# songxf1024/GIMS

Hardware: NVIDIA B200
Metric: image_pairs_per_sec_2048kp (higher is better)
Workload: dtype f32

## Files before the change

gims_b200/csrc/attention_f16.cu:

```cuda
#include <math_constants.h>

#include "common.cuh"
#include "tc_common.cuh"

namespace gims {

namespace {

using namespace tc;

constexpr int TQ = 128;
constexpr int NQT = 2;
constexpr int TKV = 64;
constexpr int HD = 64;
constexpr int kStages = 4;
constexpr int kPlaneBytes = TKV * HD * 2;
constexpr int kThreads16 = 384;

template <int PLANES> struct Cfg16 {
  static constexpr int kStageBytes = PLANES * kPlaneBytes;
  static constexpr int kSmem = 2 * kStages * kStageBytes + 1024 + 512;
};

constexpr int cS = 0, cPh = 64, cPl = 96, cO = 128, cQh = 192, cQl = 224, cTile = 256;

__device__ long long* g_attn16_trace = nullptr;

struct Attn16Args {
  const float* qp;
  float* out;
  Segs segs;
  int cross;
  int rows_total;
  int vbase[kMaxSegs];
  unsigned* status;
};

__device__ __forceinline__ float ex2_approx(float x) {
  float y;
  asm("ex2.approx.ftz.f32 %0, %1;" : "=f"(y) : "f"(x));
  return y;
}

__device__ __forceinline__ uint64_t uniform64(uint64_t x) {
  const uint32_t lo = __shfl_sync(0xffffffffu, (uint32_t)x, 0), hi = __shfl_sync(0xffffffffu, (uint32_t)(x >> 32), 0);
  return ((uint64_t)hi << 32) | lo;
}

template <int PLANES, int FMT>
__global__ void __launch_bounds__(kThreads16, 1)
k_attention_f16(const __grid_constant__ CUtensorMap mapK, const __grid_constant__ CUtensorMap mapVt, Attn16Args a) {
  extern __shared__ uint8_t smem_raw[];
  using Cfg = Cfg16<PLANES>;
  const int img = blockIdx.z, head = blockIdx.y;
  const int src = a.cross ? (img ^ 1) : img;
  const int nq = __shfl_sync(0xffffffffu, seg_count(a.segs, img), 0);
  const int nk = __shfl_sync(0xffffffffu, seg_count(a.segs, src), 0);
  const int q0 = blockIdx.x * (NQT * TQ);
  if (q0 >= nq || nk <= 0) return;
  const int nqt = (q0 + TQ < nq) ? 2 : 1;
  const int qrow0 = a.segs.base[img] + q0;
  const int krow0 = a.segs.base[src];
  const int ntiles = (nk + TKV - 1) / TKV;

  uint8_t* smem = reinterpret_cast<uint8_t*>((reinterpret_cast<uintptr_t>(smem_raw) + 1023) & ~uintptr_t(1023));
  uint8_t* k_smem = smem;
  uint8_t* v_smem = k_smem + kStages * Cfg::kStageBytes;
  uint64_t* bars = reinterpret_cast<uint64_t*>(v_smem + kStages * Cfg::kStageBytes);
  uint64_t* k_full = bars;
  uint64_t* k_empty = bars + kStages;
  uint64_t* v_full = bars + 2 * kStages;
  uint64_t* v_empty = bars + 3 * kStages;
  uint64_t* s_full = bars + 4 * kStages;
  uint64_t* s_free = s_full + 2;
  uint64_t* p_full = s_free + 2;
  uint64_t* o_full = p_full + 2;
  uint64_t* o_free = o_full + 2;
  uint64_t* q_ready = o_free + 2;
  uint64_t* skew = q_ready + 2;
  uint32_t* tmem_slot = reinterpret_cast<uint32_t*>(skew + 1);


  const int warp = threadIdx.x >> 5, lane = threadIdx.x & 31;
  constexpr int kWarpQk = 8, kWarpPv = 9;
  if (warp == kWarpQk && lane == 0) {
    tma_prefetch_desc(&mapK);
    tma_prefetch_desc(&mapVt);
    for (int s = 0; s < kStages; ++s) {
      mbar_init(&k_full[s], 1); mbar_init(&k_empty[s], nqt);
      mbar_init(&v_full[s], 1); mbar_init(&v_empty[s], nqt);
    }
    for (int t = 0; t < 2; ++t) {
      mbar_init(&s_full[t], 1); mbar_init(&s_free[t], 4);
      mbar_init(&p_full[t], 4); mbar_init(&o_full[t], 1); mbar_init(&o_free[t], 4);
      mbar_init(&q_ready[t], 4);
    }
    mbar_init(skew, 4);
    fence_barrier_init();
  }
  const int qt = warp >> 2;
  float4 qreg[HD / 4];
  if (warp < 8) {
    const int qr = q0 + TQ * qt + 32 * (warp & 3) + lane;
    const float4* p4 = reinterpret_cast<const float4*>(a.qp + (size_t)(qrow0 + TQ * qt + 32 * (warp & 3) + lane) * kD + head * HD);
#pragma unroll
    for (int i = 0; i < HD / 4; ++i) qreg[i] = (qr < nq) ? p4[i] : make_float4(0.f, 0.f, 0.f, 0.f);
  }
  if (warp == kWarpQk) tmem_alloc<512>(tmem_slot);
  tcgen05_fence_before();
  __syncthreads();
  tcgen05_fence_after();
  const uint32_t tmem = __shfl_sync(0xffffffffu, *tmem_slot, 0);

  const int wt = __shfl_sync(0xffffffffu, (warp - kWarpQk) >> 1, 0);
  if (warp >= 8) {
    if ((threadIdx.x == kWarpQk * 32 || threadIdx.x == (kWarpQk + 2) * 32) && wt < nqt) {
      const int t = wt;
      constexpr uint32_t idesc = umma_idesc_f16(TQ, TKV, FMT);
      const uint64_t dk0 = umma_desc_sw128(smem_u32(k_smem));
      const uint32_t sacc = tmem + cTile * t + cS, q_hi = tmem + cTile * t + cQh, q_lo = tmem + cTile * t + cQl;
      auto load_k = [&](int j, int s) {
        mbar_arrive_expect_tx(&k_full[s], Cfg::kStageBytes);
        for (int pl = 0; pl < PLANES; ++pl)
          tma_load_2d(k_smem + s * Cfg::kStageBytes + pl * kPlaneBytes, &mapK, &k_full[s], head * HD, pl * a.rows_total + krow0 + j * TKV);
      };
      if (t == 0)
        for (int j = 0; j < kStages && j < ntiles; ++j) load_k(j, j);
      mbar_wait(&q_ready[t], 0);
      long long* trace = (blockIdx.x | blockIdx.y | blockIdx.z) == 0 && t == 0 ? g_attn16_trace : nullptr;
      int s = 0; uint32_t ph = 0;
      for (int j = 0; j < ntiles; ++j) {
        mbar_wait(&k_full[s], ph);
        if (j > 0) mbar_wait(&s_free[t], (uint32_t)(j - 1) & 1u);
        tcgen05_fence_after();
        if (trace && j < 40) trace[j * 16 + 0] = clock64();
        const uint64_t kh = dk0 + (uint64_t)(s * (Cfg::kStageBytes >> 4)), kl = kh + (kPlaneBytes >> 4);
        if (PLANES == 2) {
#pragma unroll
          for (int ks = 0; ks < 4; ++ks) {
            umma_f16_ts(sacc, q_lo + ks * 8, kh + ks * 2, idesc, ks ? 1u : 0u);
            umma_f16_ts(sacc, q_hi + ks * 8, kl + ks * 2, idesc, 1u);
          }
        }
#pragma unroll
        for (int ks = 0; ks < 4; ++ks) umma_f16_ts(sacc, q_hi + ks * 8, kh + ks * 2, idesc, (PLANES == 2 || ks) ? 1u : 0u);
        umma_commit(&s_full[t]);
        umma_commit(&k_empty[s]);
        if (trace && j < 40) trace[j * 16 + 1] = clock64();
        if (t == 0 && j >= 1 && j - 1 + kStages < ntiles) {
          const int sp = s == 0 ? kStages - 1 : s - 1;
          mbar_wait(&k_empty[sp], (uint32_t)((j - 1) / kStages) & 1u);
          load_k(j - 1 + kStages, sp);
        }
        if (++s == kStages) { s = 0; ph ^= 1; }
      }
    } else if ((threadIdx.x == kWarpPv * 32 || threadIdx.x == (kWarpPv + 2) * 32) && wt < nqt) {
      const int t = wt;
      constexpr uint32_t idesc = umma_idesc_f16(TQ, HD, FMT);
      const uint64_t dv0 = umma_desc_sw128(smem_u32(v_smem));
      const uint32_t oacc = tmem + cTile * t + cO, p_hi = tmem + cTile * t + cPh, p_lo = tmem + cTile * t + cPl;
      auto load_v = [&](int j, int s) {
        mbar_arrive_expect_tx(&v_full[s], Cfg::kStageBytes);
        for (int pl = 0; pl < PLANES; ++pl)
          tma_load_2d(v_smem + s * Cfg::kStageBytes + pl * kPlaneBytes, &mapVt, &v_full[s], a.vbase[src] + j * TKV, pl * kD + head * HD);
      };
      if (t == 0)
        for (int j = 0; j < kStages && j < ntiles; ++j) load_v(j, j);
      long long* trace = (blockIdx.x | blockIdx.y | blockIdx.z) == 0 && t == 0 ? g_attn16_trace : nullptr;
      int s = 0; uint32_t ph = 0;
      for (int j = 0; j < ntiles; ++j) {
        mbar_wait(&v_full[s], ph);
        mbar_wait(&p_full[t], (uint32_t)j & 1u);
        if (j > 0) mbar_wait(&o_free[t], (uint32_t)(j - 1) & 1u);
        tcgen05_fence_after();
        if (trace && j < 40) trace[j * 16 + 2] = clock64();
        const uint64_t vh = dv0 + (uint64_t)(s * (Cfg::kStageBytes >> 4)), vl = vh + (kPlaneBytes >> 4);
        if (PLANES == 2) {
#pragma unroll
          for (int ks = 0; ks < 4; ++ks) {
            umma_f16_ts(oacc, p_lo + ks * 8, vh + ks * 2, idesc, ks ? 1u : 0u);
            umma_f16_ts(oacc, p_hi + ks * 8, vl + ks * 2, idesc, 1u);
          }
        }
#pragma unroll
        for (int ks = 0; ks < 4; ++ks) umma_f16_ts(oacc, p_hi + ks * 8, vh + ks * 2, idesc, (PLANES == 2 || ks) ? 1u : 0u);
        umma_commit(&o_full[t]);
        umma_commit(&v_empty[s]);
        if (trace && j < 40) trace[j * 16 + 3] = clock64();
        if (t == 0 && j >= 1 && j - 1 + kStages < ntiles) {
          const int sp = s == 0 ? kStages - 1 : s - 1;
          mbar_wait(&v_empty[sp], (uint32_t)((j - 1) / kStages) & 1u);
          load_v(j - 1 + kStages, sp);
        }
        if (++s == kStages) { s = 0; ph ^= 1; }
      }
    }
  } else {
    if (qt < nqt) {
      const uint32_t lane_base = tmem + ((uint32_t)(32 * (warp & 3)) << 16) + (uint32_t)(cTile * qt);
      const int row = q0 + TQ * qt + 32 * (warp & 3) + lane;
      bool ovf = false;
      {
        uint32_t vh[32], vl[32];
#pragma unroll
        for (int i = 0; i < HD / 4; ++i) {
          const float4 x = qreg[i];
          if (FMT == 0) ovf = ovf || fmaxf(fmaxf(fabsf(x.x), fabsf(x.y)), fmaxf(fabsf(x.z), fabsf(x.w))) >= 32768.f;
          if (PLANES == 2) {
            split16x2<FMT>(x.x, x.y, vh[2 * i], vl[2 * i]);
            split16x2<FMT>(x.z, x.w, vh[2 * i + 1], vl[2 * i + 1]);
          } else {
            vh[2 * i] = pack16<FMT>(x.x, x.y);
            vh[2 * i + 1] = pack16<FMT>(x.z, x.w);
          }
        }
        tmem_st_32x32(lane_base + cQh, vh);
        if (PLANES == 2) tmem_st_32x32(lane_base + cQl, vl);
        tmem_st_wait();
        tcgen05_fence_before();
        __syncwarp();
        if (lane == 0) mbar_arrive(&q_ready[qt]);
      }
      if (__any_sync(0xffffffffu, ovf) && lane == 0 && a.status) atomicOr(a.status, GIMS_STATUS_FP16_RANGE);
      float o[HD];
#pragma unroll
      for (int d = 0; d < HD; ++d) o[d] = 0.f;
      float m_run = -CUDART_INF_F, l_run = 0.f, alpha_prev = 0.f;
      long long* trace = ((blockIdx.x | blockIdx.y | blockIdx.z) == 0 && (threadIdx.x & 127) == 0) ? g_attn16_trace : nullptr;
      for (int j = 0; j <= ntiles; ++j) {
        float s[TKV];
        float alpha = 0.f;
        uint32_t ph_[32], pl_[32];
        if (j < ntiles) {
          if (j == 0 && qt == 1) mbar_wait(skew, 0);
          mbar_wait(&s_full[qt], (uint32_t)j & 1u);
          tcgen05_fence_after();
          if (trace && j < 40) trace[j * 16 + (qt ? 7 : 4)] = clock64();
          {
            uint32_t v0[32], v1[32];
            tmem_ld_32x32(lane_base + cS, v0);
            tmem_ld_32x32(lane_base + cS + 32, v1);
            tmem_ld_wait();
#pragma unroll
            for (int i = 0; i < 32; ++i) { s[i] = __uint_as_float(v0[i]); s[32 + i] = __uint_as_float(v1[i]); }
          }
          tcgen05_fence_before();
          __syncwarp();
          if (lane == 0) mbar_arrive(&s_free[qt]);
          if (trace && j < 40 && qt == 0) trace[j * 16 + 8] = clock64();
          const int valid = nk - j * TKV;
          if (valid < TKV) {
#pragma unroll
            for (int i = 0; i < TKV; ++i)
              if (i >= valid) s[i] = -CUDART_INF_F;
          }
          float mx8[8];
#pragma unroll
          for (int i = 0; i < 8; ++i) mx8[i] = s[i];
#pragma unroll
          for (int i = 8; i < TKV; ++i) mx8[i & 7] = fmaxf(mx8[i & 7], s[i]);
          const float mx = fmaxf(fmaxf(fmaxf(mx8[0], mx8[1]), fmaxf(mx8[2], mx8[3])), fmaxf(fmaxf(mx8[4], mx8[5]), fmaxf(mx8[6], mx8[7])));
          const float m_new = fmaxf(m_run, mx);
          if (trace && j < 40 && qt == 0) trace[j * 16 + 9] = clock64() + (long long)(__float_as_int(m_new) & 0);
          alpha = ex2_approx(m_run - m_new);
          float rs[4] = {0.f, 0.f, 0.f, 0.f};
#pragma unroll
          for (int i = 0; i < TKV; i += 4) {
#pragma unroll
            for (int q = 0; q < 4; ++q) {
              s[i + q] = ex2_approx(s[i + q] - m_new);
              rs[q] += s[i + q];
            }
          }
          l_run = l_run * alpha + ((rs[0] + rs[1]) + (rs[2] + rs[3]));
          m_run = m_new;
          if (trace && j < 40 && qt == 0) trace[j * 16 + 10] = clock64() + (long long)(__float_as_int(l_run) & 0);
          if (j == 0 && qt == 0) { __syncwarp(); if (lane == 0) mbar_arrive(skew); }
#pragma unroll
          for (int i = 0; i < 32; ++i) {
            if (PLANES == 2) split16x2<FMT>(s[2 * i], s[2 * i + 1], ph_[i], pl_[i]);
            else ph_[i] = pack16<FMT>(s[2 * i], s[2 * i + 1]);
          }
        }
        if (j > 0) {
          mbar_wait(&o_full[qt], (uint32_t)(j - 1) & 1u);
          tcgen05_fence_after();
          if (trace && j < 40 && qt == 0) trace[j * 16 + 11] = clock64();
        }
        if (j < ntiles) {
          tmem_st_32x32(lane_base + cPh, ph_);
          if (PLANES == 2) tmem_st_32x32(lane_base + cPl, pl_);
          tmem_st_wait();
          tcgen05_fence_before();
          __syncwarp();
          if (lane == 0) mbar_arrive(&p_full[qt]);
          if (trace && j < 40 && qt == 0) trace[j * 16 + 5] = clock64();
        }
        if (j > 0) {
          {
            uint32_t v0[32], v1[32];
            tmem_ld_32x32(lane_base + cO, v0);
            tmem_ld_32x32(lane_base + cO + 32, v1);
            tmem_ld_wait();
#pragma unroll
            for (int i = 0; i < 32; ++i) {
              o[i] = fmaf(o[i], alpha_prev, __uint_as_float(v0[i]));
              o[32 + i] = fmaf(o[32 + i], alpha_prev, __uint_as_float(v1[i]));
            }
          }
          tcgen05_fence_before();
          __syncwarp();
          if (lane == 0) mbar_arrive(&o_free[qt]);
          if (trace && j < 40 && qt == 0) trace[j * 16 + 6] = clock64();
        }
        alpha_prev = alpha;
      }
      if (row < nq) {
        const float inv = 1.f / l_run;
        float4* dst = reinterpret_cast<float4*>(a.out + (size_t)(a.segs.base[img] + row) * kD + head * HD);
#pragma unroll
        for (int d = 0; d < HD; d += 4) dst[d / 4] = make_float4(o[d] * inv, o[d + 1] * inv, o[d + 2] * inv, o[d + 3] * inv);
      }
      tcgen05_fence_before();
    }
  }
  __syncthreads();
  if (warp == kWarpQk) {
    tcgen05_fence_after();
    tmem_dealloc<512>(tmem);
  }
}

template <int PLANES, int FMT>
int launch16(const CUtensorMap& mK, const CUtensorMap& mV, const Attn16Args& a, dim3 grid, cudaStream_t st) {
  using Cfg = Cfg16<PLANES>;
  GIMS_CUDA_OK(cudaFuncSetAttribute(k_attention_f16<PLANES, FMT>, cudaFuncAttributeMaxDynamicSharedMemorySize, Cfg::kSmem));
  k_attention_f16<PLANES, FMT><<<grid, kThreads16, Cfg::kSmem, st>>>(mK, mV, a);
  GIMS_LAUNCH_OK();
  return GIMS_OK;
}

}

int set_attention16_trace(long long* dev_buf) {
  GIMS_CUDA_OK(cudaMemcpyToSymbol(g_attn16_trace, &dev_buf, sizeof(dev_buf)));
  return GIMS_OK;
}

int launch_attention_f16(const QkvPlanes& pl, float* out, const Segs& segs, int cross, cudaStream_t st) {
  const int rows = segs_rows(segs);
  if (pl.fmt < 0 || (pl.planes != 1 && pl.planes != 2) || pl.ldv % 8) {
    set_error("launch_attention_f16: bad plane description (fmt %d, planes %d, ldv %d)", pl.fmt, pl.planes, pl.ldv);
    return GIMS_ERR_ARG;
  }
  CUtensorMap mK, mV;
  GIMS_TRY(tc::make_tmap_16_k64(&mK, pl.kp, pl.fmt, (uint64_t)pl.planes * rows, kD, kD, TKV));
  GIMS_TRY(tc::make_tmap_16_k64(&mV, pl.vt, pl.fmt, (uint64_t)pl.planes * kD, pl.ldv, pl.ldv, HD));
  Attn16Args a;
  a.qp = pl.qp;
  a.out = out;
  a.segs = segs;
  a.cross = cross;
  a.rows_total = rows;
  for (int i = 0; i < kMaxSegs; ++i) a.vbase[i] = pl.vbase[i];
  a.status = pl.status;
  dim3 grid(cdiv(segs_nmax(segs), NQT * TQ), kHeads, segs.nseg);
  ProfScope prof(GIMS_PROF_ATTENTION, st);
  if (pl.planes == 2 && pl.fmt == 0) return launch16<2, 0>(mK, mV, a, grid, st);
  if (pl.planes == 1 && pl.fmt == 1) return launch16<1, 1>(mK, mV, a, grid, st);
  set_error("launch_attention_f16: unsupported combination planes=%d fmt=%d", pl.planes, pl.fmt);
  return GIMS_ERR_ARG;
}

}
```

gims_b200/csrc/tc_common.cuh:

```cuda
#pragma once
#include <cuda.h>
#include <cuda_runtime.h>
#include <stdint.h>

namespace gims {
namespace tc {

__device__ __forceinline__ uint32_t smem_u32(const void* p) { return (uint32_t)__cvta_generic_to_shared(p); }

__device__ __forceinline__ void mbar_init(uint64_t* bar, uint32_t count) {
  asm volatile("mbarrier.init.shared::cta.b64 [%0], %1;" ::"r"(smem_u32(bar)), "r"(count) : "memory");
}
__device__ __forceinline__ void fence_barrier_init() { asm volatile("fence.mbarrier_init.release.cluster;" ::: "memory"); }
__device__ __forceinline__ void mbar_arrive(uint64_t* bar) {
  asm volatile("mbarrier.arrive.shared::cta.b64 _, [%0];" ::"r"(smem_u32(bar)) : "memory");
}
__device__ __forceinline__ void mbar_arrive_expect_tx(uint64_t* bar, uint32_t bytes) {
  asm volatile("mbarrier.arrive.expect_tx.shared::cta.b64 _, [%0], %1;" ::"r"(smem_u32(bar)), "r"(bytes) : "memory");
}
static __device__ unsigned g_tc_timeout_flag;
static __device__ unsigned g_tc_timeout_info[4];
__device__ __forceinline__ bool mbar_try_wait(uint32_t addr, uint32_t parity) {
  uint32_t ok;
  asm volatile(
      "{\n\t.reg .pred p;\n\t"
      "mbarrier.try_wait.parity.shared::cta.b64 p, [%1], %2;\n\t"
      "selp.u32 %0, 1, 0, p;\n\t}"
      : "=r"(ok)
      : "r"(addr), "r"(parity)
      : "memory");
  return ok != 0;
}
__device__ __forceinline__ void mbar_wait(uint64_t* bar, uint32_t parity) {
  const uint32_t addr = smem_u32(bar);
  unsigned spins = 0;
  while (!mbar_try_wait(addr, parity)) {
    if (++spins > 400000u || ((spins & 255u) == 0 && *(volatile unsigned*)&g_tc_timeout_flag)) {
      if (atomicExch(&g_tc_timeout_flag, 1u) == 0u) {
        g_tc_timeout_info[0] = blockIdx.x; g_tc_timeout_info[1] = blockIdx.y | (blockIdx.z << 16);
        g_tc_timeout_info[2] = threadIdx.x; g_tc_timeout_info[3] = addr | (parity << 31);
      }
      return;
    }
  }
}

__device__ __forceinline__ void fence_proxy_async_smem() { asm volatile("fence.proxy.async.shared::cta;" ::: "memory"); }
__device__ __forceinline__ void tcgen05_fence_before() { asm volatile("tcgen05.fence::before_thread_sync;" ::: "memory"); }
__device__ __forceinline__ void tcgen05_fence_after() { asm volatile("tcgen05.fence::after_thread_sync;" ::: "memory"); }

__device__ __forceinline__ void tma_prefetch_desc(const CUtensorMap* m) {
  asm volatile("prefetch.tensormap [%0];" ::"l"(reinterpret_cast<uint64_t>(m)) : "memory");
}
__device__ __forceinline__ void tma_load_2d(void* smem_dst, const CUtensorMap* m, uint64_t* bar, int c0, int c1) {
  asm volatile(
      "cp.async.bulk.tensor.2d.shared::cluster.global.mbarrier::complete_tx::bytes [%0], [%1, {%3, %4}], [%2];" ::"r"(
          smem_u32(smem_dst)),
      "l"(reinterpret_cast<uint64_t>(m)), "r"(smem_u32(bar)), "r"(c0), "r"(c1)
      : "memory");
}

template <int COLS>
__device__ __forceinline__ void tmem_alloc(uint32_t* smem_result) {
  static_assert(COLS == 32 || COLS == 64 || COLS == 128 || COLS == 256 || COLS == 512, "TMEM columns: power of 2 >= 32");
  asm volatile("tcgen05.alloc.cta_group::1.sync.aligned.shared::cta.b32 [%0], %1;" ::"r"(smem_u32(smem_result)), "n"(COLS)
               : "memory");
  asm volatile("tcgen05.relinquish_alloc_permit.cta_group::1.sync.aligned;" ::: "memory");
}
template <int COLS>
__device__ __forceinline__ void tmem_dealloc(uint32_t taddr) {
  asm volatile("tcgen05.dealloc.cta_group::1.sync.aligned.b32 %0, %1;" ::"r"(taddr), "n"(COLS) : "memory");
}

__device__ __forceinline__ void tmem_ld_32x32(uint32_t taddr, uint32_t (&r)[32]) {
  asm volatile(
      "tcgen05.ld.sync.aligned.32x32b.x32.b32 "
      "{%0, %1, %2, %3, %4, %5, %6, %7, %8, %9, %10, %11, %12, %13, %14, %15, "
      "%16, %17, %18, %19, %20, %21, %22, %23, %24, %25, %26, %27, %28, %29, %30, %31}, [%32];"
      : "=r"(r[0]), "=r"(r[1]), "=r"(r[2]), "=r"(r[3]), "=r"(r[4]), "=r"(r[5]), "=r"(r[6]), "=r"(r[7]), "=r"(r[8]),
        "=r"(r[9]), "=r"(r[10]), "=r"(r[11]), "=r"(r[12]), "=r"(r[13]), "=r"(r[14]), "=r"(r[15]), "=r"(r[16]),
        "=r"(r[17]), "=r"(r[18]), "=r"(r[19]), "=r"(r[20]), "=r"(r[21]), "=r"(r[22]), "=r"(r[23]), "=r"(r[24]),
        "=r"(r[25]), "=r"(r[26]), "=r"(r[27]), "=r"(r[28]), "=r"(r[29]), "=r"(r[30]), "=r"(r[31])
      : "r"(taddr)
      : "memory");
}
__device__ __forceinline__ void tmem_ld_wait() { asm volatile("tcgen05.wait::ld.sync.aligned;" ::: "memory"); }

__device__ __forceinline__ uint64_t umma_desc_sw128(uint32_t smem_addr) {
  uint64_t d = 0;
  d |= (uint64_t)((smem_addr >> 4) & 0x3FFF);
  d |= (uint64_t)1 << 16;
  d |= (uint64_t)64 << 32;
  d |= (uint64_t)1 << 46;
  d |= (uint64_t)2 << 61;
  return d;
}
__host__ __device__ constexpr uint32_t umma_idesc_tf32(int m, int n) {
  return (1u << 4) | (2u << 7) | (2u << 10) | ((uint32_t)(n >> 3) << 17) | ((uint32_t)(m >> 4) << 24);
}
__device__ __forceinline__ void umma_tf32_ss(uint32_t tmem_d, uint64_t desc_a, uint64_t desc_b, uint32_t idesc,
                                             uint32_t accumulate) {
  asm volatile(
      "{\n\t.reg .pred p;\n\t"
      "setp.ne.b32 p, %4, 0;\n\t"
      "tcgen05.mma.cta_group::1.kind::tf32 [%0], %1, %2, %3, p;\n\t}" ::"r"(tmem_d),
      "l"(desc_a), "l"(desc_b), "r"(idesc), "r"(accumulate)
      : "memory");
}
__device__ __forceinline__ void tmem_st_32x32(uint32_t taddr, const uint32_t (&r)[32]) {
  asm volatile(
      "tcgen05.st.sync.aligned.32x32b.x32.b32 [%0], "
      "{%1, %2, %3, %4, %5, %6, %7, %8, %9, %10, %11, %12, %13, %14, %15, %16, "
      "%17, %18, %19, %20, %21, %22, %23, %24, %25, %26, %27, %28, %29, %30, %31, %32};" ::"r"(taddr),
      "r"(r[0]), "r"(r[1]), "r"(r[2]), "r"(r[3]), "r"(r[4]), "r"(r[5]), "r"(r[6]), "r"(r[7]), "r"(r[8]), "r"(r[9]),
      "r"(r[10]), "r"(r[11]), "r"(r[12]), "r"(r[13]), "r"(r[14]), "r"(r[15]), "r"(r[16]), "r"(r[17]), "r"(r[18]),
      "r"(r[19]), "r"(r[20]), "r"(r[21]), "r"(r[22]), "r"(r[23]), "r"(r[24]), "r"(r[25]), "r"(r[26]), "r"(r[27]),
      "r"(r[28]), "r"(r[29]), "r"(r[30]), "r"(r[31])
      : "memory");
}
__device__ __forceinline__ void tmem_st_32x16(uint32_t taddr, const uint32_t (&r)[16]) {
  asm volatile(
      "tcgen05.st.sync.aligned.32x32b.x16.b32 [%0], "
      "{%1, %2, %3, %4, %5, %6, %7, %8, %9, %10, %11, %12, %13, %14, %15, %16};" ::"r"(taddr),
      "r"(r[0]), "r"(r[1]), "r"(r[2]), "r"(r[3]), "r"(r[4]), "r"(r[5]), "r"(r[6]), "r"(r[7]), "r"(r[8]), "r"(r[9]),
      "r"(r[10]), "r"(r[11]), "r"(r[12]), "r"(r[13]), "r"(r[14]), "r"(r[15])
      : "memory");
}
__device__ __forceinline__ void tmem_st_wait() { asm volatile("tcgen05.wait::st.sync.aligned;" ::: "memory"); }

__device__ __forceinline__ void umma_tf32_ts(uint32_t tmem_d, uint32_t tmem_a, uint64_t desc_b, uint32_t idesc,
                                             uint32_t accumulate) {
  asm volatile(
      "{\n\t.reg .pred p;\n\t"
      "setp.ne.b32 p, %4, 0;\n\t"
      "tcgen05.mma.cta_group::1.kind::tf32 [%0], [%1], %2, %3, p;\n\t}" ::"r"(tmem_d),
      "r"(tmem_a), "l"(desc_b), "r"(idesc), "r"(accumulate)
      : "memory");
}
__host__ __device__ constexpr uint32_t umma_idesc_f16(int m, int n, int fmt) {
  return (1u << 4) | ((uint32_t)fmt << 7) | ((uint32_t)fmt << 10) | ((uint32_t)(n >> 3) << 17) | ((uint32_t)(m >> 4) << 24);
}
__device__ __forceinline__ void umma_f16_ts(uint32_t tmem_d, uint32_t tmem_a, uint64_t desc_b, uint32_t idesc,
                                            uint32_t accumulate) {
  asm volatile(
      "{\n\t.reg .pred p;\n\t"
      "setp.ne.b32 p, %4, 0;\n\t"
      "tcgen05.mma.cta_group::1.kind::f16 [%0], [%1], %2, %3, p;\n\t}" ::"r"(tmem_d),
      "r"(tmem_a), "l"(desc_b), "r"(idesc), "r"(accumulate)
      : "memory");
}
template <int FMT>
__device__ __forceinline__ uint32_t pack16(float lo, float hi) {
  uint32_t d;
  if (FMT == 0) asm("cvt.rn.f16x2.f32 %0, %1, %2;" : "=r"(d) : "f"(hi), "f"(lo));
  else          asm("cvt.rn.bf16x2.f32 %0, %1, %2;" : "=r"(d) : "f"(hi), "f"(lo));
  return d;
}
template <int FMT>
__device__ __forceinline__ void unpack16(uint32_t d, float& lo, float& hi) {
  if (FMT == 0) {
    asm("{\n\t.reg .f16 l, h;\n\tmov.b32 {l, h}, %2;\n\tcvt.f32.f16 %0, l;\n\tcvt.f32.f16 %1, h;\n\t}" : "=f"(lo), "=f"(hi) : "r"(d));
  } else {
    lo = __uint_as_float(d << 16);
    hi = __uint_as_float(d & 0xffff0000u);
  }
}
template <int FMT>
__device__ __forceinline__ void split16x2(float x0, float x1, uint32_t& hi, uint32_t& lo) {
  hi = pack16<FMT>(x0, x1);
  float h0, h1;
  unpack16<FMT>(hi, h0, h1);
  lo = pack16<FMT>(x0 - h0, x1 - h1);
}

__device__ __forceinline__ void umma_commit(uint64_t* bar) {
  asm volatile("tcgen05.commit.cta_group::1.mbarrier::arrive::one.shared::cluster.b64 [%0];" ::"r"(smem_u32(bar))
               : "memory");
}

__device__ __forceinline__ void split_tf32(float x, float& hi, float& lo) {
  const uint32_t h = (__float_as_uint(x) + 0x1000u) & 0xffffe000u;
  hi = __uint_as_float(h);
  lo = x - hi;
}

typedef CUresult (*EncodeTiledFn)(CUtensorMap*, CUtensorMapDataType, cuuint32_t, void*, const cuuint64_t*,
                                  const cuuint64_t*, const cuuint32_t*, const cuuint32_t*, CUtensorMapInterleave,
                                  CUtensorMapSwizzle, CUtensorMapL2promotion, CUtensorMapFloatOOBfill);
EncodeTiledFn get_encode_tiled();
int make_tmap_f32_k32(CUtensorMap* out, const float* base, uint64_t rows, uint64_t cols, uint64_t ld, uint32_t box_rows);
int make_tmap_16_k64(CUtensorMap* out, const void* base, int fmt, uint64_t rows, uint64_t cols, uint64_t ld, uint32_t box_rows);

}
}
```

Before: 664.9.

## Double KV tile to 128, alias P into S columns, interleave two Q tiles

Raises the KV tile from 64 to 128 rows and drops to 3 pipeline stages, loading V^T as two 64-column TMA boxes per stage. The softmax probabilities are now written in place over the S accumulator columns in small 32x4 chunks, which removes the separate P region and the s_free barrier. QK for the next tile now waits on o_full, and a new 'turn' barrier alternates the two Q tiles' QK issue. The intent is fewer per-tile barrier round trips and better tensor-core and softmax overlap, at the cost of less prefetch depth, stricter serialization between the S and P uses of the same TMEM, and added globaltimer tracing.

```diff
diff --git a/gims_b200/csrc/attention_f16.cu b/gims_b200/csrc/attention_f16.cu
--- a/gims_b200/csrc/attention_f16.cu
+++ b/gims_b200/csrc/attention_f16.cu
@@ -11,10 +11,12 @@
 
 constexpr int TQ = 128;
 constexpr int NQT = 2;
-constexpr int TKV = 64;
+constexpr int TKV = 128;
 constexpr int HD = 64;
-constexpr int kStages = 4;
+constexpr int kStages = 3;
+constexpr bool kSplitP = false;
 constexpr int kPlaneBytes = TKV * HD * 2;
+constexpr int kVtBoxBytes = 64 * HD * 2;
 constexpr int kThreads16 = 384;
 
 template <int PLANES> struct Cfg16 {
@@ -22,8 +24,11 @@
   static constexpr int kSmem = 2 * kStages * kStageBytes + 1024 + 512;
 };
 
-constexpr int cS = 0, cPh = 64, cPl = 96, cO = 128, cQh = 192, cQl = 224, cTile = 256;
-
+constexpr int cS = 0, cO = 128, cQh = 192, cQl = 224, cTile = 256;
+
+__host__ __device__ constexpr int p_col(int ks) { return 32 * (ks >> 1) + 8 * (ks & 1); }
+
+constexpr int kTraceCta = 63 * 16;
 __device__ long long* g_attn16_trace = nullptr;
 
 struct Attn16Args {
@@ -42,6 +47,12 @@
   return y;
 }
 
+__device__ __forceinline__ long long globaltimer() {
+  long long t;
+  asm volatile("mov.u64 %0, %%globaltimer;" : "=l"(t));
+  return t;
+}
+
 __device__ __forceinline__ uint64_t uniform64(uint64_t x) {
   const uint32_t lo = __shfl_sync(0xffffffffu, (uint32_t)x, 0), hi = __shfl_sync(0xffffffffu, (uint32_t)(x >> 32), 0);
   return ((uint64_t)hi << 32) | lo;
@@ -53,6 +64,10 @@
   extern __shared__ uint8_t smem_raw[];
   using Cfg = Cfg16<PLANES>;
   const int img = blockIdx.z, head = blockIdx.y;
+  if ((blockIdx.x | blockIdx.y | blockIdx.z | threadIdx.x) == 0 && g_attn16_trace) {
+    g_attn16_trace[kTraceCta] = globaltimer();
+    g_attn16_trace[kTraceCta + 2] = clock64();
+  }
   const int src = a.cross ? (img ^ 1) : img;
   const int nq = __shfl_sync(0xffffffffu, seg_count(a.segs, img), 0);
   const int nk = __shfl_sync(0xffffffffu, seg_count(a.segs, src), 0);
@@ -72,13 +87,12 @@
   uint64_t* v_full = bars + 2 * kStages;
   uint64_t* v_empty = bars + 3 * kStages;
   uint64_t* s_full = bars + 4 * kStages;
-  uint64_t* s_free = s_full + 2;
-  uint64_t* p_full = s_free + 2;
+  uint64_t* p_full = s_full + 2;
   uint64_t* o_full = p_full + 2;
   uint64_t* o_free = o_full + 2;
   uint64_t* q_ready = o_free + 2;
-  uint64_t* skew = q_ready + 2;
-  uint32_t* tmem_slot = reinterpret_cast<uint32_t*>(skew + 1);
+  uint64_t* turn = q_ready + 2;
+  uint32_t* tmem_slot = reinterpret_cast<uint32_t*>(turn + 2);
 
 
   const int warp = threadIdx.x >> 5, lane = threadIdx.x & 31;
@@ -91,11 +105,10 @@
       mbar_init(&v_full[s], 1); mbar_init(&v_empty[s], nqt);
     }
     for (int t = 0; t < 2; ++t) {
-      mbar_init(&s_full[t], 1); mbar_init(&s_free[t], 4);
+      mbar_init(&s_full[t], 1);
       mbar_init(&p_full[t], 4); mbar_init(&o_full[t], 1); mbar_init(&o_free[t], 4);
-      mbar_init(&q_ready[t], 4);
+      mbar_init(&q_ready[t], 4); mbar_init(&turn[t], 4);
     }
-    mbar_init(skew, 4);
     fence_barrier_init();
   }
   const int qt = warp >> 2;
@@ -131,7 +144,9 @@
       int s = 0; uint32_t ph = 0;
       for (int j = 0; j < ntiles; ++j) {
         mbar_wait(&k_full[s], ph);
-        if (j > 0) mbar_wait(&s_free[t], (uint32_t)(j - 1) & 1u);
+        if (j > 0) mbar_wait(&o_full[t], (uint32_t)(j - 1) & 1u);
+        if (t == 1) mbar_wait(&turn[0], (uint32_t)j & 1u);
+        else if (j > 0 && nqt == 2) mbar_wait(&turn[1], (uint32_t)(j - 1) & 1u);
         tcgen05_fence_after();
         if (trace && j < 40) trace[j * 16 + 0] = clock64();
         const uint64_t kh = dk0 + (uint64_t)(s * (Cfg::kStageBytes >> 4)), kl = kh + (kPlaneBytes >> 4);
@@ -158,11 +173,13 @@
       const int t = wt;
       constexpr uint32_t idesc = umma_idesc_f16(TQ, HD, FMT);
       const uint64_t dv0 = umma_desc_sw128(smem_u32(v_smem));
-      const uint32_t oacc = tmem + cTile * t + cO, p_hi = tmem + cTile * t + cPh, p_lo = tmem + cTile * t + cPl;
+      const uint32_t oacc = tmem + cTile * t + cO, p_hi = tmem + cTile * t + cS, p_lo = p_hi + 16;
       auto load_v = [&](int j, int s) {
         mbar_arrive_expect_tx(&v_full[s], Cfg::kStageBytes);
         for (int pl = 0; pl < PLANES; ++pl)
-          tma_load_2d(v_smem + s * Cfg::kStageBytes + pl * kPlaneBytes, &mapVt, &v_full[s], a.vbase[src] + j * TKV, pl * kD + head * HD);
+          for (int h = 0; h < 2; ++h)
+            tma_load_2d(v_smem + s * Cfg::kStageBytes + pl * kPlaneBytes + h * kVtBoxBytes, &mapVt, &v_full[s],
+                        a.vbase[src] + j * TKV + 64 * h, pl * kD + head * HD);
       };
       if (t == 0)
         for (int j = 0; j < kStages && j < ntiles; ++j) load_v(j, j);
@@ -170,20 +187,43 @@
       int s = 0; uint32_t ph = 0;
       for (int j = 0; j < ntiles; ++j) {
         mbar_wait(&v_full[s], ph);
-        mbar_wait(&p_full[t], (uint32_t)j & 1u);
         if (j > 0) mbar_wait(&o_free[t], (uint32_t)(j - 1) & 1u);
+        mbar_wait(&p_full[t], kSplitP ? 0u : (uint32_t)j & 1u);
         tcgen05_fence_after();
         if (trace && j < 40) trace[j * 16 + 2] = clock64();
         const uint64_t vh = dv0 + (uint64_t)(s * (Cfg::kStageBytes >> 4)), vl = vh + (kPlaneBytes >> 4);
+        const int nks = nk - j * TKV > 64 ? 8 : 4;
+        auto vofs = [](int ks) { return (uint64_t)((ks >> 2) * (kVtBoxBytes >> 4) + (ks & 3) * 2); };
+        uint32_t acc = 0u;
+        auto mma = [&](uint32_t pa, uint64_t vb) { umma_f16_ts(oacc, pa, vb, idesc, acc); acc = 1u; };
+        auto first_products = [&](int ks0, int ks1) {
+#pragma unroll
+          for (int ks = ks0; ks < ks1; ++ks) {
+            if (PLANES == 2) {
+              mma(p_lo + p_col(ks), vh + vofs(ks));
+              mma(p_hi + p_col(ks), vl + vofs(ks));
+            } else {
+              mma(p_hi + p_col(ks), vh + vofs(ks));
+            }
+          }
+        };
+        if (kSplitP) {
+          if (nks == 8) first_products(4, 8);
+          mbar_wait(&p_full[t], 1u);
+          tcgen05_fence_after();
+          first_products(0, 4);
+        } else if (nks == 8) {
+          first_products(0, 8);
+        } else {
+          first_products(0, 4);
+        }
         if (PLANES == 2) {
 #pragma unroll
-          for (int ks = 0; ks < 4; ++ks) {
-            umma_f16_ts(oacc, p_lo + ks * 8, vh + ks * 2, idesc, ks ? 1u : 0u);
-            umma_f16_ts(oacc, p_hi + ks * 8, vl + ks * 2, idesc, 1u);
-          }
-        }
-#pragma unroll
-        for (int ks = 0; ks < 4; ++ks) umma_f16_ts(oacc, p_hi + ks * 8, vh + ks * 2, idesc, (PLANES == 2 || ks) ? 1u : 0u);
+          for (int ks = 0; ks < 8; ++ks) {
+            if (ks == nks) break;
+            mma(p_hi + p_col(ks), vh + vofs(ks));
+          }
+        }
         umma_commit(&o_full[t]);
         umma_commit(&v_empty[s]);
         if (trace && j < 40) trace[j * 16 + 3] = clock64();
@@ -228,75 +268,10 @@
       float m_run = -CUDART_INF_F, l_run = 0.f, alpha_prev = 0.f;
       long long* trace = ((blockIdx.x | blockIdx.y | blockIdx.z) == 0 && (threadIdx.x & 127) == 0) ? g_attn16_trace : nullptr;
       for (int j = 0; j <= ntiles; ++j) {
-        float s[TKV];
-        float alpha = 0.f;
-        uint32_t ph_[32], pl_[32];
-        if (j < ntiles) {
-          if (j == 0 && qt == 1) mbar_wait(skew, 0);
-          mbar_wait(&s_full[qt], (uint32_t)j & 1u);
-          tcgen05_fence_after();
-          if (trace && j < 40) trace[j * 16 + (qt ? 7 : 4)] = clock64();
-          {
-            uint32_t v0[32], v1[32];
-            tmem_ld_32x32(lane_base + cS, v0);
-            tmem_ld_32x32(lane_base + cS + 32, v1);
-            tmem_ld_wait();
-#pragma unroll
-            for (int i = 0; i < 32; ++i) { s[i] = __uint_as_float(v0[i]); s[32 + i] = __uint_as_float(v1[i]); }
-          }
-          tcgen05_fence_before();
-          __syncwarp();
-          if (lane == 0) mbar_arrive(&s_free[qt]);
-          if (trace && j < 40 && qt == 0) trace[j * 16 + 8] = clock64();
-          const int valid = nk - j * TKV;
-          if (valid < TKV) {
-#pragma unroll
-            for (int i = 0; i < TKV; ++i)
-              if (i >= valid) s[i] = -CUDART_INF_F;
-          }
-          float mx8[8];
-#pragma unroll
-          for (int i = 0; i < 8; ++i) mx8[i] = s[i];
-#pragma unroll
-          for (int i = 8; i < TKV; ++i) mx8[i & 7] = fmaxf(mx8[i & 7], s[i]);
-          const float mx = fmaxf(fmaxf(fmaxf(mx8[0], mx8[1]), fmaxf(mx8[2], mx8[3])), fmaxf(fmaxf(mx8[4], mx8[5]), fmaxf(mx8[6], mx8[7])));
-          const float m_new = fmaxf(m_run, mx);
-          if (trace && j < 40 && qt == 0) trace[j * 16 + 9] = clock64() + (long long)(__float_as_int(m_new) & 0);
-          alpha = ex2_approx(m_run - m_new);
-          float rs[4] = {0.f, 0.f, 0.f, 0.f};
-#pragma unroll
-          for (int i = 0; i < TKV; i += 4) {
-#pragma unroll
-            for (int q = 0; q < 4; ++q) {
-              s[i + q] = ex2_approx(s[i + q] - m_new);
-              rs[q] += s[i + q];
-            }
-          }
-          l_run = l_run * alpha + ((rs[0] + rs[1]) + (rs[2] + rs[3]));
-          m_run = m_new;
-          if (trace && j < 40 && qt == 0) trace[j * 16 + 10] = clock64() + (long long)(__float_as_int(l_run) & 0);
-          if (j == 0 && qt == 0) { __syncwarp(); if (lane == 0) mbar_arrive(skew); }
-#pragma unroll
-          for (int i = 0; i < 32; ++i) {
-            if (PLANES == 2) split16x2<FMT>(s[2 * i], s[2 * i + 1], ph_[i], pl_[i]);
-            else ph_[i] = pack16<FMT>(s[2 * i], s[2 * i + 1]);
-          }
-        }
         if (j > 0) {
           mbar_wait(&o_full[qt], (uint32_t)(j - 1) & 1u);
           tcgen05_fence_after();
           if (trace && j < 40 && qt == 0) trace[j * 16 + 11] = clock64();
-        }
-        if (j < ntiles) {
-          tmem_st_32x32(lane_base + cPh, ph_);
-          if (PLANES == 2) tmem_st_32x32(lane_base + cPl, pl_);
-          tmem_st_wait();
-          tcgen05_fence_before();
-          __syncwarp();
-          if (lane == 0) mbar_arrive(&p_full[qt]);
-          if (trace && j < 40 && qt == 0) trace[j * 16 + 5] = clock64();
-        }
-        if (j > 0) {
           {
             uint32_t v0[32], v1[32];
             tmem_ld_32x32(lane_base + cO, v0);
@@ -313,6 +288,77 @@
           if (lane == 0) mbar_arrive(&o_free[qt]);
           if (trace && j < 40 && qt == 0) trace[j * 16 + 6] = clock64();
         }
+        if (j == ntiles) break;
+        if (j == 0 && qt == 1) mbar_wait(&turn[0], 0);
+        mbar_wait(&s_full[qt], (uint32_t)j & 1u);
+        tcgen05_fence_after();
+        if (trace && j < 40) trace[j * 16 + (qt ? 7 : 4)] = clock64();
+        const int valid = nk - j * TKV;
+        auto load_s = [&](int h, float (&x)[64]) {
+          uint32_t v0[32], v1[32];
+          tmem_ld_32x32(lane_base + cS + 64 * h, v0);
+          tmem_ld_32x32(lane_base + cS + 64 * h + 32, v1);
+          tmem_ld_wait();
+#pragma unroll
+          for (int i = 0; i < 32; ++i) { x[i] = __uint_as_float(v0[i]); x[32 + i] = __uint_as_float(v1[i]); }
+          if (valid < TKV) {
+#pragma unroll
+            for (int i = 0; i < 64; ++i)
+              if (64 * h + i >= valid) x[i] = -CUDART_INF_F;
+          }
+        };
+        float s[64];
+        float mx8[8];
+        load_s(0, s);
+#pragma unroll
+        for (int i = 0; i < 8; ++i) mx8[i] = s[i];
+#pragma unroll
+        for (int i = 8; i < 64; ++i) mx8[i & 7] = fmaxf(mx8[i & 7], s[i]);
+        load_s(1, s);
+        if (trace && j < 40 && qt == 0) trace[j * 16 + 8] = clock64();
+#pragma unroll
+        for (int i = 0; i < 64; ++i) mx8[i & 7] = fmaxf(mx8[i & 7], s[i]);
+        const float mx = fmaxf(fmaxf(fmaxf(mx8[0], mx8[1]), fmaxf(mx8[2], mx8[3])), fmaxf(fmaxf(mx8[4], mx8[5]), fmaxf(mx8[6], mx8[7])));
+        const float m_new = fmaxf(m_run, mx);
+        if (trace && j < 40 && qt == 0) trace[j * 16 + 9] = clock64() + (long long)(__float_as_int(m_new) & 0);
+        float rs[4] = {0.f, 0.f, 0.f, 0.f};
+        auto store_p = [&](int h, float (&x)[64]) {
+#pragma unroll
+          for (int g = 0; g < 8; ++g) {
+            uint32_t ph_[4], pl_[4];
+#pragma unroll
+            for (int i = 0; i < 4; ++i) {
+              const float e0 = ex2_approx(x[8 * g + 2 * i] - m_new), e1 = ex2_approx(x[8 * g + 2 * i + 1] - m_new);
+              rs[(2 * i) & 3] += e0;
+              rs[(2 * i + 1) & 3] += e1;
+              if (PLANES == 2) split16x2<FMT>(e0, e1, ph_[i], pl_[i]);
+              else ph_[i] = pack16<FMT>(e0, e1);
+            }
+            tmem_st_32x4(lane_base + cS + p_col(4 * h + g / 2) + 4 * (g & 1), ph_);
+            if (PLANES == 2) tmem_st_32x4(lane_base + cS + p_col(4 * h + g / 2) + 4 * (g & 1) + 16, pl_);
+          }
+        };
+        store_p(1, s);
+        if (kSplitP) {
+          tmem_st_wait();
+          tcgen05_fence_before();
+          __syncwarp();
+        }
+        if (lane == 0) {
+          if (kSplitP) mbar_arrive(&p_full[qt]);
+          mbar_arrive(&turn[qt]);
+        }
+        load_s(0, s);
+        store_p(0, s);
+        tmem_st_wait();
+        const float alpha = ex2_approx(m_run - m_new);
+        l_run = l_run * alpha + ((rs[0] + rs[1]) + (rs[2] + rs[3]));
+        m_run = m_new;
+        if (trace && j < 40 && qt == 0) trace[j * 16 + 10] = clock64() + (long long)(__float_as_int(l_run) & 0);
+        tcgen05_fence_before();
+        __syncwarp();
+        if (lane == 0) mbar_arrive(&p_full[qt]);
+        if (trace && j < 40 && qt == 0) trace[j * 16 + 5] = clock64();
         alpha_prev = alpha;
       }
       if (row < nq) {
@@ -328,6 +374,10 @@
   if (warp == kWarpQk) {
     tcgen05_fence_after();
     tmem_dealloc<512>(tmem);
+    if (lane == 0 && blockIdx.x + blockIdx.y + blockIdx.z == 0 && g_attn16_trace) {
+      g_attn16_trace[kTraceCta + 1] = globaltimer();
+      g_attn16_trace[kTraceCta + 3] = clock64();
+    }
   }
 }
 
diff --git a/gims_b200/csrc/tc_common.cuh b/gims_b200/csrc/tc_common.cuh
--- a/gims_b200/csrc/tc_common.cuh
+++ b/gims_b200/csrc/tc_common.cuh
@@ -126,6 +126,11 @@
       "r"(r[10]), "r"(r[11]), "r"(r[12]), "r"(r[13]), "r"(r[14]), "r"(r[15])
       : "memory");
 }
+__device__ __forceinline__ void tmem_st_32x4(uint32_t taddr, const uint32_t (&r)[4]) {
+  asm volatile("tcgen05.st.sync.aligned.32x32b.x4.b32 [%0], {%1, %2, %3, %4};" ::"r"(taddr), "r"(r[0]), "r"(r[1]), "r"(r[2]),
+               "r"(r[3])
+               : "memory");
+}
 __device__ __forceinline__ void tmem_st_wait() { asm volatile("tcgen05.wait::st.sync.aligned;" ::: "memory"); }
 
 __device__ __forceinline__ void umma_tf32_ts(uint32_t tmem_d, uint32_t tmem_a, uint64_t desc_b, uint32_t idesc,
```

Result: no change. 661.1 (median of 6 runs) (-0.6%).
